# zhibaishouheilab/HealthiVert-GAN

Measured on NVIDIA B200. Metric: slices/sec two-stage gen fwd (256x256), higher is better.
Workload: dtype bf16

## Files before the change

### healthivert-gan_b200/build.py

```python
import os
import subprocess
import sys

HERE = os.path.dirname(os.path.abspath(__file__))
CSRC = os.path.join(HERE, "csrc")
LIB = os.path.join(HERE, "libhv_b200.so")
SOURCES = ["hv_api.cu", "sn_prepare.cu", "conv_fp32.cu", "ctx_attn.cu", "mask_ops.cu", "generator_plan.cu",
           "conv_tc.cu", "conv_tc_api.cu", "gemm_tc.cu", "ctx_attn_tc.cu", "train_ops.cu", "slice_prep.cu", "resample.cu", "pipeline.cu", "trunk_tc.cu", "dconv_tc.cu", "gconv_tc.cu"]
NVCC_FLAGS = ["-gencode", "arch=compute_100a,code=sm_100a", "-lineinfo", "-O3", "-std=c++17",
              "-Xcompiler", "-fPIC", "-shared"]


def _stale():
    if not os.path.exists(LIB):
        return True
    t = os.path.getmtime(LIB)
    deps = [os.path.join(CSRC, f) for f in os.listdir(CSRC)]
    deps.append(os.path.join(os.path.dirname(HERE), "include", "hv_b200.h"))
    return any(os.path.getmtime(d) > t for d in deps)


def build(force=False, verbose=False):
    if not force and not _stale():
        return LIB
    nvcc = os.environ.get("NVCC", "/usr/local/cuda/bin/nvcc")
    objs = []
    procs = []
    os.makedirs(os.path.join(HERE, "build"), exist_ok=True)
    for src in SOURCES:
        obj = os.path.join(HERE, "build", src.replace(".cu", ".o"))
        cmd = [nvcc] + NVCC_FLAGS[:-1] + ["-c", os.path.join(CSRC, src), "-o", obj]
        if verbose:
            cmd.insert(1, "-Xptxas=-v")
        procs.append((src, subprocess.Popen(cmd, stdout=subprocess.PIPE, stderr=subprocess.STDOUT, text=True)))
        objs.append(obj)
    for src, p in procs:
        out, _ = p.communicate()
        if verbose and out:
            print(out)
        if p.returncode != 0:
            raise RuntimeError(f"nvcc failed on {src}:\n{out}")
    cmd = [nvcc, "-gencode", "arch=compute_100a,code=sm_100a", "-shared", "-o", LIB] + objs
    r = subprocess.run(cmd, stdout=subprocess.PIPE, stderr=subprocess.STDOUT, text=True)
    if r.returncode != 0:
        raise RuntimeError(f"link failed:\n{r.stdout}")
    return LIB


if __name__ == "__main__":
    print(build(force="--force" in sys.argv, verbose="-v" in sys.argv))
```

### healthivert-gan_b200/csrc/conv_tc.cu

```cuda
#include <stdlib.h>
#include <string.h>
#include <vector>
#include "hv_common.cuh"
#include "conv_tc.cuh"
#include "tc_ptx.cuh"

namespace hv {

__device__ __forceinline__ float exp_neg_fast(float x) {
  float y;
  asm("ex2.approx.ftz.f32 %0, %1;" : "=f"(y) : "f"(x * 1.4426950408889634f));
  return y;
}

template <int ACT>
__device__ __forceinline__ float act_fast(float x, int act_rt) {
  if (ACT == HV_ACT_ELU) return x > 0.f ? x : exp_neg_fast(x) - 1.f;
  if (ACT == HV_ACT_RELU) return fmaxf(x, 0.f);
  switch (act_rt) {
    case HV_ACT_ELU: return x > 0.f ? x : __expf(x) - 1.f;
    case HV_ACT_RELU: return fmaxf(x, 0.f);
    case HV_ACT_SIGMOID: return 1.f / (1.f + __expf(-x));
    case HV_ACT_LRELU02: return x > 0.f ? x : 0.2f * x;
    case HV_ACT_CLAMP1: return fminf(fmaxf(x, -1.f), 1.f);
// ... 740 lines not shown
        const int ky = (ch >> 2) - py, kx = (ch & 3) - px;
        if (entry == 1 && ch < 16 && ky >= 0 && ky < 3 && kx >= 0 && kx < 3) v = wa[((size_t)co * cin_total + s.ch_off) * kk + ky * 3 + kx];
      } else if (ch < s.real) {
        const int dy = entry / 3 - 1, dx = entry % 3 - 1;
        for (int ky = 0; ky < 3; ++ky)
          for (int kx = 0; kx < 3; ++kx)
            if (((py + ky - 1) >> 1) == dy && ((px + kx - 1) >> 1) == dx) v += wa[((size_t)co * cin_total + s.ch_off + ch) * kk + ky * 3 + kx];
      }
    }
    dst[i] = __float2bfloat16(v);
    return;
  }
  if (real) {
    const int cin = s.ch_off + c;
    if (co < cout_a) v = wa[((size_t)co * cin_total + cin) * kk + tap];
    else if (co < cout_a + cout_b) v = wb[((size_t)(co - cout_a) * cin_total + cin) * kk + tap];
  }
  dst[i] = __float2bfloat16(v);
}

int tc_conv_pack_weights(TcConv& c, const float* wa, const float* ba, int cout_a, const float* wb, const float* bb,
                         int cout_b, cudaStream_t st) {
  HV_CHECK_ARG(cout_a + cout_b == c.cout_real, "tc_conv_pack_weights: filter count mismatch");
  PackSrc s0, s1;
  memset(&s0, 0, sizeof(s0)); memset(&s1, 0, sizeof(s1));
  s0.real = c.src[0].real_channels; s0.chunks = c.src[0].buf.chunks; s0.kxpack = c.src[0].kxpack ? 1 : 0; s0.xp = c.p.in_xp; s0.cp = c.p.cp;
  s1.chunks = 1; s1.xp = 1;
  s0.ups = c.p.ups;
  if (c.p.ups) HV_CHECK_ARG(cout_b == 0, "tc_conv_pack_weights: the sub-pixel upsample mode takes one filter bank");
  if (c.src[0].chan_map) {
    HV_CHECK_ARG(c.src[0].kxpack && c.src[0].buf.chunks * 8 <= 32, "tc_conv_pack_weights: a channel map needs a kx-packed source of <= 32 channels");
    s0.use_map = 1;
    for (int i = 0; i < 32; ++i) s0.map[i] = i < c.src[0].buf.chunks * 8 ? c.src[0].chan_map[i] : (short)-1;
  }
  int cin_total = c.src[0].real_channels;
  if (c.nsrc == 2) {
    s1.ch_off = c.src[0].real_channels; s1.real = c.src[1].real_channels; s1.chunks = c.src[1].buf.chunks; s1.kxpack = c.src[1].kxpack ? 1 : 0;
    s1.nbhd4 = c.src[1].nbhd4 ? 1 : 0;
    cin_total += c.src[1].real_channels;
  }
  const int total = (int)(c.p.w_bytes / 2);
  pack_weights_kernel<<<(max(total, c.n_pad) + 255) / 256, 256, 0, st>>>(wa, ba, cout_a, wb, bb, cout_b, cin_total, c.k, c.n_pad, s0,
                                                                          s1, c.nsrc, (__nv_bfloat16*)c.w_packed, c.bias_pad, total);
  HV_LAUNCH_CHECK();
  return HV_OK;
}

static long long* g_trace = nullptr;
static bool g_pdl = getenv("HV_NO_PDL") == nullptr;
void tc_set_trace(long long* dev_buf) { g_trace = dev_buf; }
static long long* g_timeline = nullptr;
static int g_timeline_count = 0;
void tc_set_timeline(long long* dev_buf) { g_timeline = dev_buf; g_timeline_count = 0; }

template <int N_PAD, int ACT, int FIXED = 0, bool DIAG = true>
static int tc_launch_na(const TcConv& c, cudaStream_t st) {
  static bool configured = false;
  if (!configured) {
    HV_CUDA(cudaFuncSetAttribute(conv_tc_kernel<N_PAD, ACT, FIXED, DIAG>, cudaFuncAttributeMaxDynamicSharedMemorySize, 227 * 1024));
    configured = true;
  }
  cudaLaunchConfig_t cfg = {};
  cfg.gridDim = dim3(c.grid);
  cfg.blockDim = dim3(tc_threads(N_PAD));
  cfg.dynamicSmemBytes = c.smem;
  cfg.stream = st;
  cudaLaunchAttribute attr[1];
  attr[0].id = cudaLaunchAttributeProgrammaticStreamSerialization;
  attr[0].val.programmaticStreamSerializationAllowed = 1;
  cfg.attrs = attr;
  cfg.numAttrs = g_pdl ? 1 : 0;
  TcParams q = c.p;
  q.trace = g_trace;
  q.timeline = g_timeline ? g_timeline + 4 * (g_timeline_count++) : nullptr;
  HV_CUDA(cudaLaunchKernelEx(&cfg, conv_tc_kernel<N_PAD, ACT, FIXED, DIAG>, q));
  HV_LAUNCH_CHECK();
  return HV_OK;
}

static int tc_issue_code(const TcConv& c);
static int tc_fixed_code(const TcConv& c) {
  if (c.force_generic) return 0;
  const int issue = tc_issue_code(c);
  if (!issue) return 0;
  const TcParams& p = c.p;
  int out = 0;
  if (p.out_mode == TC_OUT_HEADS) out = 3;
  else if (p.out_mode == TC_OUT_CHUNKED_S2D) out = 4;
  else if (p.out_mode == TC_OUT_CHUNKED) out = p.out_xp > 1 ? 5 : 1;
  else out = p.out_xp > 1 ? 6 : 2;
  return (p.pair ? 1 << 20 : 0) | out << 16 | issue;
}
static int tc_issue_code(const TcConv& c) {
  const TcParams& p = c.p;
  static const bool no_fixed = getenv("HV_TC_NO_FIXED") != nullptr;
  if (no_fixed) return 0;
  const TcSeg& s0 = p.segs[0];
  const int ks = s0.nchunks >> 1;
  if (p.s2d_in) return p.nseg == 1 ? tc_shape_code(2, 0, 0, ks) : 0;
  if (p.in_xp > 1) {
    for (int i = 1; i < p.nseg; ++i)
      if (p.segs[i].nrows != s0.nrows || p.segs[i].nchunks != s0.nchunks) return 0;
    return tc_shape_code(3, s0.nrows, 0, ks);
  }
  if (p.nseg == 2 && s0.nrows == 3 && s0.ntaps == 3 && p.segs[1].nrows == 3 && p.segs[1].ntaps == 1 && p.segs[1].nchunks == 2)
    return tc_shape_code(4, 0, 0, ks);
// ... 300 lines not shown
```

### healthivert-gan_b200/csrc/conv_tc.cuh

```cuda
#pragma once
#include <cuda.h>
#include <cuda_bf16.h>
#include <cuda_runtime.h>
#include <stdint.h>

namespace hv {

struct TcBuf {
  __nv_bfloat16* ptr = nullptr;
  int n = 0, chunks = 0, h = 0, w = 0, border = 0;
  bool s2d = false;
  int xp = 1;
  int img_chunks = 0;
  __host__ __device__ int image_chunks() const { return img_chunks ? img_chunks : chunks; }
  __host__ __device__ size_t chunk_base(int i, int c) const { return ((size_t)i * image_chunks() + c) * (size_t)plane() * 8; }
  TcBuf chunk_view(int c0, int count) const {
    TcBuf v = *this;
    v.img_chunks = image_chunks();
    v.ptr = ptr + (size_t)c0 * plane() * 8;
    v.chunks = count;
    return v;
  }
  __host__ __device__ int sub_h() const { return s2d ? h / 2 : h; }
  __host__ __device__ int sub_w() const { return s2d ? w / 2 : w / xp; }
// ... 60 lines not shown
  int out_mode;
  __nv_bfloat16* out;
  int out_pitch, out_border, out_plane, out_sub_plane, out_chunks_total, out_chunk_off, out_nchunks;
  float* head0;
  float* head1;
  TcAux aux0, aux1;
  uint32_t slot_bytes;
  int nslots;
  long long* trace;
  long long* timeline;
  int debug;
};

struct TcSource {
  TcBuf buf;
  int real_channels;
  bool kxpack = false;
  const short* chan_map = nullptr;
  bool nbhd4 = false;
};

struct TcConv {
  TcParams p;
  int n_pad = 0;
  int grid = 0;
  int ctas_per_sm = 1;
  size_t smem = 0;
  void* w_packed = nullptr;
  float* bias_pad = nullptr;
  int k = 0, stride = 1, dil = 1;
  int nsrc = 0;
  TcSource src[2];
  int cout_real = 0;
  bool force_generic = false;
  void* arena = nullptr;
  static constexpr size_t kArenaBytes = 4u << 20;
};

int tc_conv_setup(TcConv& c, const TcSource* srcs, int nsrc, int k, int stride, int dil, int cout_real,
                  int n_images, bool allow_pair = false, bool ups = false);
void tc_conv_set_batch(TcConv& c, int n_images);
int tc_conv_pack_weights(TcConv& c, const float* w_eff_a, const float* bias_a, int cout_a, const float* w_eff_b,
                         const float* bias_b, int cout_b, cudaStream_t st);
void tc_conv_set_output_chunked(TcConv& c, const TcBuf& out, int chunk_off, int nchunks, bool up2, int act);
void tc_conv_set_output_heads(TcConv& c, float* head0, float* head1, const TcAux* aux0, const TcAux* aux1);
int tc_conv_launch(const TcConv& c, cudaStream_t st);
void tc_set_trace(long long* dev_buf);
void tc_conv_free(TcConv& c);

bool tc_trunk_eligible(const TcConv& c);
size_t tc_trunk_counter_ints(int max_images);
int tc_trunk_launch(const TcConv* const* convs, int count, int n_images, int* counters, cudaStream_t st);

int tc_pack_nchw(const float* src, int src_channels, int mode , const TcBuf& dst, int dst_channel0,
                 cudaStream_t st);
struct TcPlaneSrc { const float* ptr; int mode; };
int tc_pack_kx(const TcPlaneSrc* srcs, int nsrc, int k, int dil, const TcBuf& dst, cudaStream_t st);
int tc_pack_nbhd4(const float* src, const TcBuf& dst, cudaStream_t st);
int tc_unpack_nchw(const TcBuf& src, int channel0, int channels, float* dst, cudaStream_t st, int sub = 1);
int tc_gap_fc_sigmoid(const TcBuf& x, const float* fc_w, const float* fc_b, float* out, float* partial ,
                      unsigned int* ticket , cudaStream_t st);

void tc_set_timeline(long long* dev_buf);
size_t ctx_attn_tc_workspace_bytes(int n);
int ctx_attn_fwd_tc(const TcBuf& f, const float* mask, const TcBuf& y, int32_t* offsets, float* flow, float scale, int fuse,
                    int per_sample_mask, void* workspace, cudaStream_t st, cudaStream_t st_aux = nullptr, cudaEvent_t* evs = nullptr);

}
```

### healthivert-gan_b200/csrc/generator_plan.cu

```cuda
#include <string.h>
#include <vector>
#include "hv_common.cuh"
#include "kernels.h"
#include "conv_tc.cuh"

namespace hv {

struct LayerSpec {
  const char* name;
  int cin, cout, k, stride, pad, dil, act, hout;
};

static const LayerSpec kLayers[] = {
    {"coarse_generator.conv1", 3, 16, 5, 1, 2, 1, HV_ACT_ELU, 256},
    {"coarse_generator.conv2_downsample", 16, 32, 3, 2, 1, 1, HV_ACT_ELU, 128},
    {"coarse_generator.conv3", 32, 32, 3, 1, 1, 1, HV_ACT_ELU, 128},
    {"coarse_generator.conv4_downsample", 32, 64, 3, 2, 1, 1, HV_ACT_ELU, 64},
    {"coarse_generator.conv5", 64, 64, 3, 1, 1, 1, HV_ACT_ELU, 64},
    {"coarse_generator.conv6", 64, 64, 3, 1, 1, 1, HV_ACT_ELU, 64},
    {"coarse_generator.conv7_atrous", 64, 64, 3, 1, 2, 2, HV_ACT_ELU, 64},
    {"coarse_generator.conv8_atrous", 64, 64, 3, 1, 4, 4, HV_ACT_ELU, 64},
    {"coarse_generator.conv9_atrous", 64, 64, 3, 1, 8, 8, HV_ACT_ELU, 64},
    {"coarse_generator.conv10_atrous", 64, 64, 3, 1, 16, 16, HV_ACT_ELU, 64},
    {"coarse_generator.conv11", 64, 64, 3, 1, 1, 1, HV_ACT_ELU, 64},
// ... 177 lines not shown
    {32, 128, 1}, {16, 128, 1}, {32, 256, 1}, {16, 256, 1}, {16, 256, 1},
    {32, 256, 2}, {32, 256, 1}, {16, 128, 1}, {32, 128, 1}, {32, 64, 1}, {64, 64, 1}, {64, 64, 2}, {64, 64, 4},
    {64, 64, 8}, {64, 64, 16}, {64, 64, 1},
    {0, 256, 1}, {16, 128, 1}, {32, 128, 1}, {64, 64, 1}, {64, 64, 1}, {64, 64, 1}, {64, 64, 1}, {64, 64, 1}, {64, 64, 1},
    {64, 64, 1}, {64, 64, 1}, {64, 64, 1}, {32, 128, 1}, {32, 128, 1}, {16, 256, 1}, {16, 256, 1},
};

struct TcLayerSpec { int layer; int src0, real0, src1, real1; int out; bool up2; int out_chunks; bool kx0, kx1; bool ups; };
static const TcLayerSpec kTcLayers[] = {
    {C1, B_IN_C, 3, -1, 0, B_C1, false, 2, true, false},  {C2, B_C1, 16, -1, 0, B_C2, false, 4},
    {C3, B_C2, 32, -1, 0, B_C3, false, 4},      {C4, B_C3, 32, -1, 0, B_C4, false, 8},
    {C5, B_C4, 64, -1, 0, B_C5, false, 8},      {C6, B_C5, 64, -1, 0, B_C6, false, 8},
    {C7, B_C6, 64, -1, 0, B_C7, false, 8},      {C8, B_C7, 64, -1, 0, B_C8, false, 8},
    {C9, B_C8, 64, -1, 0, B_C9, false, 8},      {C10, B_C9, 64, -1, 0, B_C10, false, 8},
    {C11, B_C10, 64, -1, 0, B_C11, false, 8},   {C12, B_C11, 64, -1, 0, B_C12U, true, 8},
    {C20, B_C12U, 64, B_CAM128, 1, B_C20, false, 8, false, true}, {C13, B_C20, 64, -1, 0, B_C13, false, 4},
    {C14, B_C13, 32, -1, 0, B_C14, false, 4},   {C19, B_C14, 32, B_CAM4, 1, B_C19, false, 4, false, true, true},
    {C15, B_C19, 32, -1, 0, B_C15, false, 2},   {C16, B_C15, 16, -1, 0, B_C16, false, 2},
    {C17, B_C16, 8, -1, 0, -1, false, 0},
    {F1, B_IN_F, 4, -1, 0, B_F1, false, 4, true, false},  {F2, B_F1, 16, -1, 0, B_F2, false, 2},
    {F3, B_F2, 16, -1, 0, B_F3, false, 4},      {F4, B_F3, 32, -1, 0, B_F4, false, 4},
    {F5, B_F4, 32, -1, 0, B_F5, false, 8},      {F6, B_F5, 64, -1, 0, B_F6, false, 8},
    {F7, B_F6, 64, -1, 0, B_F7, false, 8},      {F8, B_F7, 64, -1, 0, B_F8, false, 8},
    {F9, B_F8, 64, -1, 0, B_F9, false, 8},      {F10, B_F9, 64, -1, 0, B_F10, false, 8},
    {PM2, B_P1, 16, -1, 0, B_P2, false, 2},
    {PM3, B_P2, 16, -1, 0, B_P3, false, 4},     {PM4, B_P3, 32, -1, 0, B_P4, false, 8},
    {PM5, B_P4, 64, -1, 0, B_P5, false, 8},     {PM6, B_P5, 64, -1, 0, B_P6, false, 8},
    {PM9, B_CA, 64, -1, 0, B_P9, false, 8},     {PM10, B_P9, 64, -1, 0, B_P10, false, 8},
    {A11, B_F10, 64, B_P10, 64, B_A11, false, 8}, {A12, B_A11, 64, -1, 0, B_A12, false, 8},
    {A19, B_A12, 64, -1, 0, B_A19, false, 8},   {A13, B_A19, 64, -1, 0, B_A13, false, 4, false, false, true},
    {A14, B_A13, 32, -1, 0, B_A14, false, 4},   {A15, B_A14, 32, -1, 0, B_A15, false, 2, false, false, true},
    {A16, B_A15, 16, -1, 0, B_A16CAT, false, 1},
    {A17, B_A16CAT, 9, -1, 0, -1, false, 0},
};
constexpr int kNumTcLayers = sizeof(kTcLayers) / sizeof(kTcLayers[0]);

static const short kFineInputMap[32] = {
    0 * 64 + 0, 0 * 64 + 2, 0 * 64 + 3, 1 * 64 + 0, 1 * 64 + 2, 1 * 64 + 3, 2 * 64 + 0, 2 * 64 + 2, 2 * 64 + 3, 3 * 64 + 0, 3 * 64 + 2, 3 * 64 + 3,
    4 * 64 + 0, 4 * 64 + 2, 4 * 64 + 3, -1,
    0 * 64 + 1, 1 * 64 + 1, 2 * 64 + 1, 3 * 64 + 1, 4 * 64 + 1, -1, -1, -1, -1, -1, -1, -1, -1, -1, -1, -1};

struct TcPlan {
  TcBuf buf[B_COUNT];
  TcConv conv[kNumLayers];
  bool has[kNumLayers] = {};
  int out_buf[kNumLayers];
  bool out_up2[kNumLayers] = {};
  void* ca_ws = nullptr;
  float* gap_partial = nullptr;
  unsigned int* gap_ticket = nullptr;
  __nv_bfloat16* blob = nullptr;
  int* trunk_ctr = nullptr;
  size_t trunk_ctr_stride = 0;
};

static int run_layers(hv_generator* g, const int* layers, int count, int n, cudaStream_t st) {
  TcPlan* t = g->tc;
  static const int force = getenv("HV_TRUNK") ? atoi(getenv("HV_TRUNK")) : 0;
  static const int min_batch = getenv("HV_TRUNK_MIN_BATCH") ? atoi(getenv("HV_TRUNK_MIN_BATCH")) : (1 << 30);
  bool ok = (force == 1 || n >= min_batch) && count >= 2 && count <= 8;
  const TcConv* convs[8];
  for (int i = 0; i < count; ++i) {
    tc_conv_set_batch(t->conv[layers[i]], n);
    if (ok) { convs[i] = &t->conv[layers[i]]; ok = tc_trunk_eligible(*convs[i]) && (i == count - 1 || !t->out_up2[layers[i]]); }
  }
  if (ok) return tc_trunk_launch(convs, count, n, t->trunk_ctr + (size_t)layers[0] * t->trunk_ctr_stride, st);
  for (int i = 0; i < count; ++i) {
    int rc = tc_conv_launch(t->conv[layers[i]], st);
    if (rc) return rc;
  }
  return HV_OK;
}

static TcAux make_aux(const TcBuf& b, int channel) {
  TcAux a;
  a.ptr = b.ptr; a.chunks = b.chunks; a.chunk = channel >> 3; a.channel = channel & 7;
  a.pitch = b.pitch(); a.border = b.border; a.plane = b.plane(); a.sub_plane = b.sub_plane();
  return a;
}

static void tc_plan_destroy(hv_generator* g) {
  if (!g->tc) return;
  for (int i = 0; i < kNumLayers; ++i) if (g->tc->has[i]) tc_conv_free(g->tc->conv[i]);
  cudaFree(g->tc->blob); cudaFree(g->tc->ca_ws); cudaFree(g->tc->gap_partial); cudaFree(g->tc->gap_ticket); cudaFree(g->tc->trunk_ctr);
  delete g->tc;
  g->tc = nullptr;
}

static int tc_plan_create(hv_generator* g) {
  TcPlan* t = new TcPlan();
  g->tc = t;
  const int n = g->max_batch;
  size_t total = 0;
  const bool no_xp = getenv("HV_NO_XP") != nullptr;
  for (int i = 0; i < B_COUNT; ++i) {
    TcBuf& b = t->buf[i];
    b.n = n; b.chunks = kBufs[i].channels / 8; b.h = b.w = kBufs[i].extent; b.border = kBufs[i].border;
    b.s2d = (i == B_C1 || i == B_C3 || i == B_F1 || i == B_F3 || i == B_P1 || i == B_P3);
    b.xp = (!no_xp && (i == B_C19 || i == B_C15 || i == B_C16 || i == B_A15 || i == B_A16CAT)) ? 4 : 1;
    total += (b.bytes() + 255) & ~(size_t)255;
  }
  total += TcBuf::kSlackBytes;
  HV_CUDA(cudaMalloc((void**)&t->blob, total));
  HV_CUDA(cudaMemset(t->blob, 0, total));
  size_t off = 0;
  for (int i = 0; i < B_COUNT; ++i) {
    t->buf[i].ptr = reinterpret_cast<__nv_bfloat16*>(reinterpret_cast<char*>(t->blob) + off);
    off += (t->buf[i].bytes() + 255) & ~(size_t)255;
  }
  t->buf[B_P1] = t->buf[B_F1].chunk_view(2, 2);
  HV_CUDA(cudaMalloc(&t->ca_ws, ctx_attn_tc_workspace_bytes(n)));
  HV_CUDA(cudaMalloc((void**)&t->gap_partial, sizeof(float) * 2 * n * 8));
  HV_CUDA(cudaMalloc((void**)&t->gap_ticket, sizeof(unsigned int) * 2 * n));
  HV_CUDA(cudaMemset(t->gap_ticket, 0, sizeof(unsigned int) * 2 * n));
  t->trunk_ctr_stride = tc_trunk_counter_ints(n);
  HV_CUDA(cudaMalloc((void**)&t->trunk_ctr, sizeof(int) * t->trunk_ctr_stride * kNumLayers));
  HV_CUDA(cudaMemset(t->trunk_ctr, 0, sizeof(int) * t->trunk_ctr_stride * kNumLayers));
  for (int i = 0; i < kNumLayers; ++i) t->out_buf[i] = -1;
  t->out_buf[PM1] = B_P1;
  for (int i = 0; i < kNumTcLayers; ++i) {
    const TcLayerSpec& s = kTcLayers[i];
    const LayerSpec& L = kLayers[s.layer];
    TcSource srcs[2];
    srcs[0].buf = s.layer == F2 ? t->buf[B_F1].chunk_view(0, 2) : t->buf[s.src0];
    srcs[0].real_channels = s.real0; srcs[0].kxpack = s.kx0;
    if (s.layer == F1) srcs[0].chan_map = kFineInputMap;
    int nsrc = 1;
    if (s.src1 >= 0) { srcs[1].buf = t->buf[s.src1]; srcs[1].real_channels = s.real1; srcs[1].kxpack = s.kx1; srcs[1].nbhd4 = s.ups; nsrc = 2; }
    const bool heads = s.out < 0;
    TcConv& c = t->conv[s.layer];
    const int cout = heads ? 2 : (s.layer == F1 ? kLayers[F1].cout + kLayers[PM1].cout : L.cout);
    int rc = tc_conv_setup(c, srcs, nsrc, L.k, L.stride, L.dil, cout, n, true, s.ups);
    if (rc) return rc;
    t->has[s.layer] = true;
    if (heads) {
      TcAux a0 = make_aux(t->buf[B_A16CAT], 8);
      tc_conv_set_output_heads(c, nullptr, nullptr, s.layer == C17 ? &a0 : nullptr, nullptr);
    } else {
      tc_conv_set_output_chunked(c, t->buf[s.out], 0, s.out_chunks, s.up2, L.act);
      t->out_buf[s.layer] = s.out; t->out_up2[s.layer] = s.up2;
    }
  }
  return HV_OK;
}

static void tc_set_batch(TcConv& c, int n) { tc_conv_set_batch(c, n); }

static int tc_plan_pack_weights(hv_generator* g, cudaStream_t st) {
  TcPlan* t = g->tc;
  for (int i = 0; i < kNumTcLayers; ++i) {
    const int l = kTcLayers[i].layer;
    int rc;
    if (kTcLayers[i].out < 0)
      rc = tc_conv_pack_weights(t->conv[l], g->w_eff[l], g->bias[l], 1, g->w_eff[l + 1], g->bias[l + 1], 1, st);
    else if (l == F1)
      rc = tc_conv_pack_weights(t->conv[l], g->w_eff[F1], g->bias[F1], kLayers[F1].cout, g->w_eff[PM1], g->bias[PM1], kLayers[PM1].cout, st);
    else
      rc = tc_conv_pack_weights(t->conv[l], g->w_eff[l], g->bias[l], kLayers[l].cout, nullptr, nullptr, 0, st);
    if (rc) return rc;
  }
  return HV_OK;
}

static int forward_bf16(hv_generator* g, const float* x, const float* mask, const float* cam, const float* ratio, int n,
                        float* coarse_seg, float* fine_seg, float* x_stage1, float* x_stage2, float* flow, float* pred1_h,
                        float* pred2_h, int32_t* offsets, int per_sample_mask, cudaStream_t st) {
  TcPlan* t = g->tc;
  auto view = [&](int id) { TcBuf b = t->buf[id]; b.n = n; return b; };
  auto run = [&](int layer, cudaStream_t s) -> int {
    TcConv& c = t->conv[layer];
    tc_set_batch(c, n);
    return tc_conv_launch(c, s);
  };
  static const bool use_aux = getenv("HV_NO_AUX_STREAM") == nullptr;
  cudaStream_t ax = use_aux ? g->aux : st;
  auto fork_aux = [&](int ev) -> int {
    if (!use_aux) return HV_OK;
    HV_CUDA(cudaEventRecord(g->ev_aux[ev], st));
    HV_CUDA(cudaStreamWaitEvent(ax, g->ev_aux[ev], 0));
    return HV_OK;
  };
  auto join_aux = [&](int ev) -> int {
    if (!use_aux) return HV_OK;
    HV_CUDA(cudaEventRecord(g->ev_aux[ev], ax));
    HV_CUDA(cudaStreamWaitEvent(st, g->ev_aux[ev], 0));
    return HV_OK;
  };
  {
    RC(fork_aux(0));
    const TcPlaneSrc in_c[3] = {{x, HV_SRC_DIRECT}, {ratio, HV_SRC_SCALAR}, {mask, HV_SRC_DIRECT}};
    RC(tc_pack_kx(in_c, 3, 5, 1, view(B_IN_C), st));
    const TcPlaneSrc cam128[1] = {{cam, HV_SRC_SUB2}};
    RC(tc_pack_kx(cam128, 1, 3, 1, view(B_CAM128), ax));
    RC(tc_pack_nbhd4(cam, view(B_CAM4), ax));
    const TcPlaneSrc in_f0[3] = {{x, HV_SRC_DIRECT}, {mask, HV_SRC_DIRECT}, {ratio, HV_SRC_SCALAR}};
    RC(tc_pack_kx(in_f0, 3, 5, 1, view(B_IN_F).chunk_view(0, 2), ax));
    if (use_aux) HV_CUDA(cudaEventRecord(g->ev_aux[1], ax));
  }
  auto chain = [&](std::initializer_list<int> ls, cudaStream_t s) -> int { return run_layers(g, ls.begin(), (int)ls.size(), n, s); };
  for (int l : {C1, C2, C3, C4}) RC(run(l, st));
  RC(chain({C5, C6, C7, C8, C9, C10, C11, C12}, st));
  RC(fork_aux(2));
  RC(tc_gap_fc_sigmoid(view(B_C10), g->fc_w[0], g->fc_b[0], pred1_h, t->gap_partial, t->gap_ticket, ax));
  if (use_aux) HV_CUDA(cudaStreamWaitEvent(st, g->ev_aux[1], 0));
  for (int l : {C20, C13, C14, C19, C15, C16}) RC(run(l, st));
  t->conv[C17].p.head0 = x_stage1; t->conv[C17].p.head1 = coarse_seg;
  RC(run(C17, st));
  {
    const TcPlaneSrc in_f1[1] = {{coarse_seg, HV_SRC_DIRECT}};
    RC(tc_pack_kx(in_f1, 1, 5, 1, view(B_IN_F).chunk_view(2, 2), st));
  }
  RC(run(F1, st));
  HV_CUDA(cudaEventRecord(g->ev_fork, st));
  HV_CUDA(cudaStreamWaitEvent(g->side, g->ev_fork, 0));
  cudaStream_t sa = g->side;
  for (int l : {PM2, PM3, PM4}) RC(run(l, sa));
  RC(chain({PM5, PM6}, sa));
  RC(ctx_attn_fwd_tc(view(B_P6), mask, view(B_CA), offsets, flow, 10.f, 1, per_sample_mask, t->ca_ws, sa, use_aux ? ax : nullptr,
                     use_aux ? &g->ev_aux[6] : nullptr));
  RC(chain({PM9, PM10}, sa));
  HV_CUDA(cudaEventRecord(g->ev_join, sa));
  for (int l : {F2, F3, F4, F5}) RC(run(l, st));
  RC(chain({F6, F7, F8, F9, F10}, st));
  HV_CUDA(cudaStreamWaitEvent(st, g->ev_join, 0));
  RC(run(A11, st));
  RC(fork_aux(4));
  RC(tc_gap_fc_sigmoid(view(B_A11), g->fc_w[1], g->fc_b[1], pred2_h, t->gap_partial + g->max_batch * 8, t->gap_ticket + g->max_batch, ax));
  RC(chain({A12, A19}, st));
  for (int l : {A13, A14, A15, A16}) RC(run(l, st));
  t->conv[A17].p.head0 = x_stage2; t->conv[A17].p.head1 = fine_seg;
  RC(run(A17, st));
  RC(join_aux(5));
  g->last_heads[0] = x_stage1; g->last_heads[1] = coarse_seg; g->last_heads[2] = x_stage2; g->last_heads[3] = fine_seg;
  g->last_n = n;
  return HV_OK;
}

}

extern "C" {

int hv_generator_num_layers(void) { return kNumLayers; }

int hv_generator_layer_info(int idx, char* name_out, int* cin, int* cout, int* k, int* stride, int* pad, int* dil,
                            int* act) {
  HV_CHECK_ARG(idx >= 0 && idx < kNumLayers, "layer_info: index %d out of range", idx);
  const LayerSpec& L = kLayers[idx];
  if (name_out) { strncpy(name_out, L.name, 63); name_out[63] = 0; }
  if (cin) *cin = L.cin;
  if (cout) *cout = L.cout;
  if (k) *k = L.k;
  if (stride) *stride = L.stride;
  if (pad) *pad = L.pad;
  if (dil) *dil = L.dil;
  if (act) *act = L.act;
  return HV_OK;
}

int hv_generator_destroy(hv_generator* g) {
  if (!g) return HV_OK;
  tc_plan_destroy(g);
  for (int i = 0; i < kNumLayers; ++i) cudaFree(g->act[i]);
  cudaFree(g->ca_out); cudaFree(g->ca_ws); cudaFree(g->sigma); cudaFree(g->d_jobs);
  cudaFree(g->blob_w); cudaFree(g->blob_b);
  if (g->side) cudaStreamDestroy(g->side);
  if (g->ev_fork) cudaEventDestroy(g->ev_fork);
  if (g->ev_join) cudaEventDestroy(g->ev_join);
  if (g->aux) cudaStreamDestroy(g->aux);
  for (cudaEvent_t e : g->ev_aux) if (e) cudaEventDestroy(e);
  delete g;
  return HV_OK;
}

int hv_generator_create(hv_generator** out, int max_batch, int precision) {
  HV_CHECK_ARG(out, "generator_create: null out pointer");
  HV_CHECK_ARG(max_batch >= 1 && max_batch <= 4096, "generator_create: max_batch %d out of range", max_batch);
  HV_CHECK_ARG(precision == HV_PREC_FP32 || precision == HV_PREC_BF16, "generator_create: bad precision %d", precision);
  int ndev = 0;
  HV_CUDA(cudaGetDeviceCount(&ndev));
  hv_generator* g = new hv_generator();
  g->max_batch = max_batch; g->precision = precision;
  size_t wtot = 0, btot = 0;
  for (int i = 0; i < kNumLayers; ++i) { wtot += (size_t)kLayers[i].cout * kLayers[i].cin * kLayers[i].k * kLayers[i].k; btot += kLayers[i].cout; }
#define GEN_TRY(expr) do { cudaError_t _e = (expr); if (_e != cudaSuccess) { hv::set_error("%s failed: %s", #expr, cudaGetErrorString(_e)); hv_generator_destroy(g); return HV_ERR_CUDA; } } while (0)
// ... 76 lines not shown
    return forward_bf16(g, x, mask, cam, ratio, n, coarse_seg, fine_seg, x_stage1, x_stage2, flow, pred1_h, pred2_h,
                        offsets, per_sample_mask, as_stream(stream));
  return forward_fp32(g, x, mask, cam, ratio, n, coarse_seg, fine_seg, x_stage1, x_stage2, flow, pred1_h, pred2_h,
                      offsets, per_sample_mask, as_stream(stream));
}

int hv_generator_run_layer(hv_generator* g, int idx, int n, hv_stream_t stream) {
  HV_CHECK_ARG(g && g->tc, "generator_run_layer: needs a bf16 plan");
  if (!g->prepared) { set_error("generator_run_layer: call hv_generator_prepare first"); return HV_ERR_STATE; }
  HV_CHECK_ARG(idx >= 0 && idx < kNumLayers && g->tc->has[idx] && g->tc->out_buf[idx] >= 0,
               "generator_run_layer: layer %d is not a stand-alone tensor-core conv", idx);
  HV_CHECK_ARG(n >= 1 && n <= g->max_batch, "generator_run_layer: batch %d outside 1..%d", n, g->max_batch);
  tc_set_batch(g->tc->conv[idx], n);
  return tc_conv_launch(g->tc->conv[idx], as_stream(stream));
}

int hv_generator_run_chain(hv_generator* g, int first, int count, int n, hv_stream_t stream) {
  HV_CHECK_ARG(g && g->tc, "generator_run_chain: needs a bf16 plan");
  if (!g->prepared) { set_error("generator_run_chain: call hv_generator_prepare first"); return HV_ERR_STATE; }
  HV_CHECK_ARG(n >= 1 && n <= g->max_batch && count >= 1 && first >= 0 && first + count <= kNumLayers, "generator_run_chain: bad range");
  int layers[kNumLayers];
  for (int idx = first; idx < first + count; ++idx) {
    HV_CHECK_ARG(g->tc->has[idx] && g->tc->out_buf[idx] >= 0, "generator_run_chain: layer %d is not a stand-alone tensor-core conv", idx);
    layers[idx - first] = idx;
  }
  return run_layers(g, layers, count, n, as_stream(stream));
}

long long hv_generator_read_tap(hv_generator* g, int idx, float* out, hv_stream_t stream) {
  HV_CHECK_ARG(g && out, "generator_read_tap: null argument");
  HV_CHECK_ARG(g->last_n > 0, "generator_read_tap: no forward has run");
  const float* src = nullptr;
  size_t count = 0;
  if (idx == kTapAttention && g->tc) {
    TcBuf v = g->tc->buf[B_CA];
    v.n = g->last_n;
    int rc = tc_unpack_nchw(v, 0, 64, out, as_stream(stream));
    if (rc) return rc;
    return (long long)g->last_n * 64 * 64 * 64;
  }
  if (idx == kTapAttention) { src = g->ca_out; count = (size_t)g->last_n * 64 * 64 * 64; }
  else {
    HV_CHECK_ARG(idx >= 0 && idx < kNumLayers, "generator_read_tap: index %d out of range", idx);
    count = act_elems(idx, g->last_n);
    if (idx == C17) src = g->last_heads[0];
    else if (idx == C18) src = g->last_heads[1];
    else if (idx == A17) src = g->last_heads[2];
    else if (idx == A18) src = g->last_heads[3];
    else if (g->tc) {
      const int b = g->tc->out_buf[idx];
      HV_CHECK_ARG(b >= 0, "generator_read_tap: layer %d has no tap in bf16 mode", idx);
      TcBuf v = g->tc->buf[b];
      v.n = g->last_n;
      const int ch = idx == A16 ? 8 : kLayers[idx].cout;
      int rc = tc_unpack_nchw(v, 0, ch, out, as_stream(stream), g->tc->out_up2[idx] ? 2 : 1);
      if (rc) return rc;
      return (long long)count;
    }
    else src = g->act[idx];
  }
  HV_CUDA(cudaMemcpyAsync(out, src, count * sizeof(float), cudaMemcpyDeviceToDevice, as_stream(stream)));
  return (long long)count;
}

}
```

Baseline: 20520.

## Fuse final 3x3 conv and dual heads into one warp-specialized tcgen05 tail kernel

Adds a persistent tail kernel that computes the last mid 3x3 ELU conv and the dual-head 3x3 conv (tanh-clamp and sigmoid) back to back. The intermediate activation stays in shared memory ring slots instead of going through global memory. The kernel also writes the kx-packed coarse segmentation for the refinement stage, which removes the separate pack_kx launch. Both stages of the generator use it by default. Tap reads of the fused mid layers now recompute them on demand, and the tight pipeline adds synchronization complexity and correctness risk.

```diff
diff --git a/healthivert-gan_b200/build.py b/healthivert-gan_b200/build.py
--- a/healthivert-gan_b200/build.py
+++ b/healthivert-gan_b200/build.py
@@ -6,7 +6,7 @@
 CSRC = os.path.join(HERE, "csrc")
 LIB = os.path.join(HERE, "libhv_b200.so")
 SOURCES = ["hv_api.cu", "sn_prepare.cu", "conv_fp32.cu", "ctx_attn.cu", "mask_ops.cu", "generator_plan.cu",
-           "conv_tc.cu", "conv_tc_api.cu", "gemm_tc.cu", "ctx_attn_tc.cu", "train_ops.cu", "slice_prep.cu", "resample.cu", "pipeline.cu", "trunk_tc.cu", "dconv_tc.cu", "gconv_tc.cu"]
+           "conv_tc.cu", "conv_tc_api.cu", "gemm_tc.cu", "ctx_attn_tc.cu", "train_ops.cu", "slice_prep.cu", "resample.cu", "pipeline.cu", "trunk_tc.cu", "tail_tc.cu", "dconv_tc.cu", "gconv_tc.cu"]
 NVCC_FLAGS = ["-gencode", "arch=compute_100a,code=sm_100a", "-lineinfo", "-O3", "-std=c++17",
               "-Xcompiler", "-fPIC", "-shared"]
 
diff --git a/healthivert-gan_b200/csrc/conv_tc.cu b/healthivert-gan_b200/csrc/conv_tc.cu
--- a/healthivert-gan_b200/csrc/conv_tc.cu
+++ b/healthivert-gan_b200/csrc/conv_tc.cu
@@ -816,6 +816,8 @@
 static long long* g_timeline = nullptr;
 static int g_timeline_count = 0;
 void tc_set_timeline(long long* dev_buf) { g_timeline = dev_buf; g_timeline_count = 0; }
+bool tc_pdl_enabled() { return g_pdl; }
+long long* tc_timeline_next() { return g_timeline ? g_timeline + 4 * (g_timeline_count++) : nullptr; }
 
 template <int N_PAD, int ACT, int FIXED = 0, bool DIAG = true>
 static int tc_launch_na(const TcConv& c, cudaStream_t st) {
diff --git a/healthivert-gan_b200/csrc/conv_tc.cuh b/healthivert-gan_b200/csrc/conv_tc.cuh
--- a/healthivert-gan_b200/csrc/conv_tc.cuh
+++ b/healthivert-gan_b200/csrc/conv_tc.cuh
@@ -136,6 +136,33 @@
 size_t tc_trunk_counter_ints(int max_images);
 int tc_trunk_launch(const TcConv* const* convs, int count, int n_images, int* counters, cudaStream_t st);
 
+struct TcTailParams {
+  CUtensorMap maps[4];
+  const void* w_mid;
+  const void* w_head;
+  const float* bias_mid;
+  const float* bias_head;
+  int n, h, w_img;
+  int rows_per_unit, strips, units;
+  float* head0;
+  float* head1;
+  TcAux aux0;
+  TcBuf kx;
+  int kx_chunk;
+  long long* timeline;
+};
+struct TcTail {
+  TcTailParams p;
+  int grid = 0;
+};
+int tc_tail_setup(TcTail& t, const TcConv& mid, const TcConv& heads, int n_images);
+void tc_tail_set_batch(TcTail& t, int n_images);
+void tc_tail_set_outputs(TcTail& t, float* head0, float* head1);
+int tc_tail_set_kxpack(TcTail& t, const TcBuf* dst, int chunk);
+int tc_tail_launch(const TcTail& t, cudaStream_t st);
+bool tc_pdl_enabled();
+long long* tc_timeline_next();
+
 int tc_pack_nchw(const float* src, int src_channels, int mode , const TcBuf& dst, int dst_channel0,
                  cudaStream_t st);
 struct TcPlaneSrc { const float* ptr; int mode; };
diff --git a/healthivert-gan_b200/csrc/generator_plan.cu b/healthivert-gan_b200/csrc/generator_plan.cu
--- a/healthivert-gan_b200/csrc/generator_plan.cu
+++ b/healthivert-gan_b200/csrc/generator_plan.cu
@@ -253,7 +253,14 @@
   __nv_bfloat16* blob = nullptr;
   int* trunk_ctr = nullptr;
   size_t trunk_ctr_stride = 0;
-};
+  TcTail tail[2];
+  bool tail_fused_last = false;
+};
+
+static bool tail_fuse_enabled() {
+  static const bool on = !(getenv("HV_NO_TAIL_FUSE") && atoi(getenv("HV_NO_TAIL_FUSE")) != 0) && !getenv("HV_NO_XP");
+  return on;
+}
 
 static int run_layers(hv_generator* g, const int* layers, int count, int n, cudaStream_t st) {
   TcPlan* t = g->tc;
@@ -341,6 +348,12 @@
       tc_conv_set_output_chunked(c, t->buf[s.out], 0, s.out_chunks, s.up2, L.act);
       t->out_buf[s.layer] = s.out; t->out_up2[s.layer] = s.up2;
     }
+  }
+  if (tail_fuse_enabled()) {
+    int rc = tc_tail_setup(t->tail[0], t->conv[C16], t->conv[C17], n);
+    if (!rc) rc = tc_tail_setup(t->tail[1], t->conv[A16], t->conv[A17], n);
+    if (!rc) rc = tc_tail_set_kxpack(t->tail[0], &t->buf[B_IN_F], 2);
+    if (rc) return rc;
   }
   return HV_OK;
 }
@@ -404,10 +417,20 @@
   RC(fork_aux(2));
   RC(tc_gap_fc_sigmoid(view(B_C10), g->fc_w[0], g->fc_b[0], pred1_h, t->gap_partial, t->gap_ticket, ax));
   if (use_aux) HV_CUDA(cudaStreamWaitEvent(st, g->ev_aux[1], 0));
-  for (int l : {C20, C13, C14, C19, C15, C16}) RC(run(l, st));
-  t->conv[C17].p.head0 = x_stage1; t->conv[C17].p.head1 = coarse_seg;
-  RC(run(C17, st));
-  {
+  const bool fuse_tail = tail_fuse_enabled();
+  auto tail = [&](int which, int conv, int heads, float* head0, float* head1) -> int {
+    if (fuse_tail) {
+      tc_tail_set_batch(t->tail[which], n);
+      tc_tail_set_outputs(t->tail[which], head0, head1);
+      return tc_tail_launch(t->tail[which], st);
+    }
+    RC(run(conv, st));
+    t->conv[heads].p.head0 = head0; t->conv[heads].p.head1 = head1;
+    return run(heads, st);
+  };
+  for (int l : {C20, C13, C14, C19, C15}) RC(run(l, st));
+  RC(tail(0, C16, C17, x_stage1, coarse_seg));
+  if (!fuse_tail) {
     const TcPlaneSrc in_f1[1] = {{coarse_seg, HV_SRC_DIRECT}};
     RC(tc_pack_kx(in_f1, 1, 5, 1, view(B_IN_F).chunk_view(2, 2), st));
   }
@@ -428,9 +451,9 @@
   RC(fork_aux(4));
   RC(tc_gap_fc_sigmoid(view(B_A11), g->fc_w[1], g->fc_b[1], pred2_h, t->gap_partial + g->max_batch * 8, t->gap_ticket + g->max_batch, ax));
   RC(chain({A12, A19}, st));
-  for (int l : {A13, A14, A15, A16}) RC(run(l, st));
-  t->conv[A17].p.head0 = x_stage2; t->conv[A17].p.head1 = fine_seg;
-  RC(run(A17, st));
+  for (int l : {A13, A14, A15}) RC(run(l, st));
+  RC(tail(1, A16, A17, x_stage2, fine_seg));
+  t->tail_fused_last = fuse_tail;
   RC(join_aux(5));
   g->last_heads[0] = x_stage1; g->last_heads[1] = coarse_seg; g->last_heads[2] = x_stage2; g->last_heads[3] = fine_seg;
   g->last_n = n;
@@ -613,6 +636,11 @@
       HV_CHECK_ARG(b >= 0, "generator_read_tap: layer %d has no tap in bf16 mode", idx);
       TcBuf v = g->tc->buf[b];
       v.n = g->last_n;
+      if (g->tc->tail_fused_last && (idx == C16 || idx == A16)) {
+        tc_set_batch(g->tc->conv[idx], g->last_n);
+        int rc = tc_conv_launch(g->tc->conv[idx], as_stream(stream));
+        if (rc) return rc;
+      }
       const int ch = idx == A16 ? 8 : kLayers[idx].cout;
       int rc = tc_unpack_nchw(v, 0, ch, out, as_stream(stream), g->tc->out_up2[idx] ? 2 : 1);
       if (rc) return rc;
diff --git a/healthivert-gan_b200/csrc/tail_tc.cu b/healthivert-gan_b200/csrc/tail_tc.cu
--- /dev/null
+++ b/healthivert-gan_b200/csrc/tail_tc.cu
@@ -0,0 +1,418 @@
+#include <string.h>
+#include "hv_common.cuh"
+#include "conv_tc.cuh"
+#include "tc_ptx.cuh"
+
+namespace hv {
+
+namespace {
+
+constexpr int kMidN = 32, kHeadN = 16;
+constexpr uint32_t kWMid = 3u * 6u * 2u * kMidN * 16u;
+constexpr uint32_t kWHead = 3u * 6u * 2u * kHeadN * 16u;
+constexpr uint32_t kSlot = 6u * 2u * 2u * 64u * 16u;
+constexpr int kSlots = 4;
+constexpr uint32_t kOffIn = kWMid + kWHead;
+constexpr uint32_t kOffMid = kOffIn + kSlots * kSlot;
+constexpr uint32_t kOffBar = kOffMid + kSlots * kSlot;
+constexpr uint32_t kOffKx = kOffBar + 1024;
+constexpr int kKxRow = 264;
+constexpr uint32_t kSmem = kOffKx + 2u * 2u * kKxRow * 4u;
+static_assert(kSmem <= 227u * 1024u, "tail kernel shared memory");
+constexpr uint32_t kInTx = kSlot;
+constexpr uint32_t kAuxTx = kSlot / 2;
+constexpr int kThreads = 20 * 32;
+constexpr int kTmemCols = 128;
+
+__device__ __forceinline__ float elu_fast(float x) {
+  if (x > 0.f) return x;
+  float y;
+  asm("ex2.approx.ftz.f32 %0, %1;" : "=f"(y) : "f"(x * 1.4426950408889634f));
+  return y - 1.f;
+}
+
+template <int N>
+__device__ __forceinline__ void issue_rows(bool leader, uint32_t d_tmem, const uint32_t (&a_lo)[3], uint32_t a_view, uint32_t b_lo) {
+  constexpr uint32_t desc_hi = (128u >> 4) | (1u << 14);
+  constexpr uint32_t idesc = (1u << 4) | (1u << 7) | (1u << 10) | ((uint32_t)(N >> 3) << 17) | ((128u >> 4) << 24);
+  constexpr uint32_t slab = 2u * N;
+  if (leader) {
+#pragma unroll
+    for (int ky = 0; ky < 3; ++ky)
+#pragma unroll
+      for (int v = 0; v < 6; ++v)
+        umma_bf16(d_tmem, ((uint64_t)desc_hi << 32) | (a_lo[ky] + (uint32_t)v * a_view),
+                  ((uint64_t)desc_hi << 32) | (b_lo + (uint32_t)(ky * 6 + v) * slab), idesc, (ky | v) == 0 ? 0u : 1u);
+  }
+}
+
+}
+
+__global__ void __launch_bounds__(kThreads, 1) tail_tc_kernel(const __grid_constant__ TcTailParams p) {
+  extern __shared__ __align__(1024) uint8_t smem[];
+  const int warp = threadIdx.x >> 5, lane = threadIdx.x & 31;
+  constexpr int W_PRODUCER = 16, W_MMA = 17, W_HEADS = 18, W_AUX = 19;
+  const uint32_t s_base = smem_u32(smem);
+  const uint32_t bars = s_base + kOffBar;
+  const uint32_t bar_in_full = bars, bar_in_empty = bars + 8 * kSlots;
+  const uint32_t bar_mid_ready = bars + 16 * kSlots, bar_mid_free = bars + 24 * kSlots;
+  const uint32_t bar_mfull = bars + 32 * kSlots, bar_mempty = bar_mfull + 16, bar_hfull = bar_mfull + 32, bar_hempty = bar_mfull + 48;
+  const uint32_t bar_w = bar_mfull + 64;
+  uint32_t* tmem_slot = reinterpret_cast<uint32_t*>(smem + kOffBar + 256);
+  float* s_bias = reinterpret_cast<float*>(smem + kOffBar + 512);
+
+  if (p.timeline && threadIdx.x == 0) {
+    unsigned long long gt;
+    asm volatile("mov.u64 %0, %%globaltimer;" : "=l"(gt));
+    atomicMin(reinterpret_cast<unsigned long long*>(p.timeline), gt);
+  }
+  if ((warp == W_PRODUCER || warp == W_AUX) && lane == 0) {
+    for (int i = 0; i < 4; ++i) asm volatile("prefetch.tensormap [%0];" ::"l"(&p.maps[i]) : "memory");
+  }
+  if (warp == W_MMA) {
+    if (lane == 0) {
+      for (int i = 0; i < kSlots; ++i) {
+        mbar_init(bar_in_full + 8u * i, 1);
+        mbar_init(bar_in_empty + 8u * i, 1);
+        mbar_init(bar_mid_ready + 8u * i, 128 + 1);
+        mbar_init(bar_mid_free + 8u * i, 1);
+      }
+      for (int i = 0; i < 2; ++i) {
+        mbar_init(bar_mfull + 8u * i, 1); mbar_init(bar_mempty + 8u * i, 128);
+        mbar_init(bar_hfull + 8u * i, 1); mbar_init(bar_hempty + 8u * i, 128);
+      }
+      mbar_init(bar_w, 1);
+      fence_barrier_init();
+    }
+    __syncwarp();
+    asm volatile("tcgen05.alloc.cta_group::1.sync.aligned.shared::cta.b32 [%0], %1;" ::"r"(smem_u32(tmem_slot)), "r"(kTmemCols) : "memory");
+    asm volatile("tcgen05.relinquish_alloc_permit.cta_group::1.sync.aligned;" ::: "memory");
+  }
+  if (threadIdx.x < kMidN) s_bias[threadIdx.x] = __ldg(p.bias_mid + threadIdx.x);
+  else if (threadIdx.x < kMidN + kHeadN) s_bias[threadIdx.x] = __ldg(p.bias_head + threadIdx.x - kMidN);
+  if (threadIdx.x < kSlots * 2 * 2) {
+    const int slot = threadIdx.x >> 2, s = (threadIdx.x >> 1) & 1, e = threadIdx.x & 1;
+    *reinterpret_cast<uint4*>(smem + kOffMid + slot * kSlot + (e ? 5 * 2048 + s * 1024 + 63 * 16 : s * 1024)) = make_uint4(0, 0, 0, 0);
+    fence_proxy_async();
+  }
+  if (threadIdx.x >= 64 && threadIdx.x < 64 + 2 * 2 * 8) {
+    const int r = (threadIdx.x - 64) >> 3, e = (threadIdx.x - 64) & 7;
+    reinterpret_cast<float*>(smem + kOffKx)[r * kKxRow + (e < 4 ? e : kKxRow - 8 + e)] = 0.f;
+  }
+  tc_fence_before();
+  __syncthreads();
+  tc_fence_after();
+  const uint32_t tmem_base = *tmem_slot;
+  asm volatile("griddepcontrol.launch_dependents;" ::: "memory");
+
+  const int R = p.rows_per_unit, strips = p.strips, units = p.units, h = p.h;
+
+  if (warp == W_PRODUCER || warp == W_AUX) {
+    const bool leader = elect_one();
+    const bool in_role = warp == W_PRODUCER;
+    if (leader && in_role) {
+      mbar_expect_tx(bar_w, kWMid + kWHead);
+      bulk_load(s_base, p.w_mid, kWMid, bar_w);
+      bulk_load(s_base + kWMid, p.w_head, kWHead, bar_w);
+    }
+    asm volatile("griddepcontrol.wait;" ::: "memory");
+    uint32_t in_seq = 0, mid_seq = 0;
+    for (int u = blockIdx.x; u < units; u += gridDim.x) {
+      const int pair = u / strips, y0 = (u - pair * strips) * R, ru = min(R, h - y0), img = 2 * pair;
+      for (int i = -2; i <= ru + 1; ++i) {
+        if (in_role) {
+          const uint32_t slot = in_seq % kSlots, par = (in_seq / kSlots) & 1u;
+          mbar_wait(bar_in_empty + 8u * slot, par ^ 1u);
+          if (leader) {
+            const uint32_t fb = bar_in_full + 8u * slot, dst = s_base + kOffIn + slot * kSlot;
+            const int row = y0 + i + 1;
+            mbar_expect_tx(fb, kInTx);
+            tma_load_5d(dst + 4096u, &p.maps[0], fb, 2, img, row, 0, 0);
+            tma_load_5d(dst, &p.maps[1], fb, 0, img, row, 0, 3);
+            tma_load_5d(dst + 5u * 4096u, &p.maps[1], fb, 4, img, row, 0, 0);
+          }
+          ++in_seq;
+        }
+        const int j = i - 1;
+        if (!in_role && j >= -1) {
+          const uint32_t slot = mid_seq % kSlots, par = (mid_seq / kSlots) & 1u;
+          mbar_wait(bar_mid_free + 8u * slot, par ^ 1u);
+          if (leader) {
+            const uint32_t fb = bar_mid_ready + 8u * slot, dst = s_base + kOffMid + slot * kSlot + 12288u;
+            const int row = y0 + j + 1;
+            mbar_expect_tx(fb, kAuxTx);
+            tma_load_5d(dst + 2048u, &p.maps[2], fb, 2, img, row, 1, 0);
+            tma_load_5d(dst, &p.maps[3], fb, 0, img, row, 1, 3);
+            tma_load_5d(dst + 5u * 2048u, &p.maps[3], fb, 4, img, row, 1, 0);
+          }
+          ++mid_seq;
+        }
+      }
+    }
+  } else if (warp == W_MMA || warp == W_HEADS) {
+    const bool leader = elect_one();
+    const bool conv_role = warp == W_MMA;
+    mbar_wait(bar_w, 0);
+    tc_fence_after();
+    const uint32_t b_mid = ((uint32_t)kMidN << 16) + (s_base >> 4);
+    const uint32_t b_head = ((uint32_t)kHeadN << 16) + ((s_base + kWMid) >> 4);
+    const uint32_t a_in = ((2048u >> 4) << 16) + ((s_base + kOffIn) >> 4);
+    const uint32_t a_mid = ((12288u >> 4) << 16) + ((s_base + kOffMid) >> 4);
+    uint32_t in_base = 0, mid_base = 0, waited = 0, cnt = 0;
+    for (int u = blockIdx.x; u < units; u += gridDim.x) {
+      const int pair = u / strips, y0 = (u - pair * strips) * R, ru = min(R, h - y0);
+      if (conv_role) {
+        for (int j = -1; j <= ru; ++j, ++cnt) {
+          while (waited < in_base + (uint32_t)(j + 4)) {
+            mbar_wait(bar_in_full + 8u * (waited % kSlots), (waited / kSlots) & 1u);
+            ++waited;
+          }
+          const uint32_t acc = cnt & 1u;
+          mbar_wait(bar_mempty + 8u * acc, ((cnt >> 1) & 1u) ^ 1u);
+          tc_fence_after();
+          uint32_t a_lo[3];
+#pragma unroll
+          for (int ky = 0; ky < 3; ++ky) a_lo[ky] = a_in + ((in_base + (uint32_t)(j + 1 + ky)) % kSlots) * (kSlot >> 4);
+          issue_rows<kMidN>(leader, tmem_base + acc * kMidN, a_lo, 4096u >> 4, b_mid);
+          if (leader) {
+            umma_commit(bar_mfull + 8u * acc);
+            umma_commit(bar_in_empty + 8u * ((in_base + (uint32_t)(j + 1)) % kSlots));
+            if (j == ru) {
+              umma_commit(bar_in_empty + 8u * ((in_base + (uint32_t)(j + 2)) % kSlots));
+              umma_commit(bar_in_empty + 8u * ((in_base + (uint32_t)(j + 3)) % kSlots));
+            }
+          }
+          __syncwarp();
+        }
+      } else {
+        for (int k = 0; k < ru; ++k, ++cnt) {
+          while (waited < mid_base + (uint32_t)(k + 3)) {
+            mbar_wait(bar_mid_ready + 8u * (waited % kSlots), (waited / kSlots) & 1u);
+            ++waited;
+          }
+          const uint32_t acc = cnt & 1u;
+          mbar_wait(bar_hempty + 8u * acc, ((cnt >> 1) & 1u) ^ 1u);
+          tc_fence_after();
+          uint32_t a_lo[3];
+#pragma unroll
+          for (int ky = 0; ky < 3; ++ky) a_lo[ky] = a_mid + ((mid_base + (uint32_t)(k + ky)) % kSlots) * (kSlot >> 4);
+          issue_rows<kHeadN>(leader, tmem_base + 2 * kMidN + acc * kHeadN, a_lo, 2048u >> 4, b_head);
+          if (leader) {
+            umma_commit(bar_hfull + 8u * acc);
+            umma_commit(bar_mid_free + 8u * ((mid_base + (uint32_t)k) % kSlots));
+            if (k == ru - 1) {
+              umma_commit(bar_mid_free + 8u * ((mid_base + (uint32_t)(k + 1)) % kSlots));
+              umma_commit(bar_mid_free + 8u * ((mid_base + (uint32_t)(k + 2)) % kSlots));
+            }
+          }
+          __syncwarp();
+        }
+      }
+      in_base += (uint32_t)(ru + 4);
+      mid_base += (uint32_t)(ru + 2);
+    }
+  } else {
+    const int quad = warp & 3, m = quad * 32 + lane, s = m >> 6, q = m & 63;
+    const uint32_t lane_off = (uint32_t)(quad * 32) << 16;
+    const bool mid_role = warp < 8;
+    const uint32_t group = (uint32_t)((warp >> 2) & 1);
+    uint32_t cnt = 0;
+    for (int u = blockIdx.x; u < units; u += gridDim.x) {
+      const int pair = u / strips, y0 = (u - pair * strips) * R, ru = min(R, h - y0);
+      const int img = 2 * pair + s;
+      if (mid_role) {
+        for (int j = -1; j <= ru; ++j, ++cnt) {
+          if ((cnt & 1u) != group) continue;
+          mbar_wait(bar_mfull + 8u * group, (cnt >> 1) & 1u);
+          tc_fence_after();
+          float v[kMidN];
+          tmem_ld<32>(tmem_base + lane_off + group * kMidN, v);
+          tmem_ld_wait();
+          tc_fence_before();
+          mbar_arrive(bar_mempty + 8u * group);
+          const int y = y0 + j;
+          const bool inside = y >= 0 && y < h;
+          uint4 val[4];
+#pragma unroll
+          for (int ph = 0; ph < 4; ++ph) {
+            uint32_t pk[4];
+#pragma unroll
+            for (int e = 0; e < 4; ++e) {
+              const int col = ph * 8 + 2 * e;
+              __nv_bfloat162 hv2 = __floats2bfloat162_rn(elu_fast(v[col] + s_bias[col]), elu_fast(v[col + 1] + s_bias[col + 1]));
+              pk[e] = inside ? *reinterpret_cast<uint32_t*>(&hv2) : 0u;
+            }
+            val[ph] = make_uint4(pk[0], pk[1], pk[2], pk[3]);
+          }
+          const uint32_t slot = cnt % kSlots;
+          mbar_wait(bar_mid_free + 8u * slot, ((cnt / kSlots) & 1u) ^ 1u);
+          uint8_t* base = smem + kOffMid + slot * kSlot + s * 1024 + q * 16;
+#pragma unroll
+          for (int ph = 0; ph < 4; ++ph) *reinterpret_cast<uint4*>(base + (ph + 1) * 2048) = val[ph];
+          if (q < 63) *reinterpret_cast<uint4*>(base + 16) = val[3];
+          if (q > 0) *reinterpret_cast<uint4*>(base + 5 * 2048 - 16) = val[0];
+          fence_proxy_async();
+          mbar_arrive(bar_mid_ready + 8u * slot);
+        }
+      } else {
+        for (int k = 0; k < ru; ++k, ++cnt) {
+          if ((cnt & 1u) != group) continue;
+          mbar_wait(bar_hfull + 8u * group, (cnt >> 1) & 1u);
+          tc_fence_after();
+          float v[kHeadN];
+          tmem_ld<16>(tmem_base + lane_off + 2 * kMidN + group * kHeadN, v);
+          tmem_ld_wait();
+          tc_fence_before();
+          mbar_arrive(bar_hempty + 8u * group);
+          const bool live = img < p.n;
+          const int y = y0 + k;
+          float seg[4];
+#pragma unroll
+          for (int jx = 0; jx < 4; ++jx) {
+            const int x = 4 * q + jx;
+            const float a0 = fminf(fmaxf(v[jx * 4] + s_bias[kMidN + jx * 4], -1.f), 1.f);
+            const float a1 = 1.f / (1.f + __expf(-(v[jx * 4 + 1] + s_bias[kMidN + jx * 4 + 1])));
+            seg[jx] = a1;
+            if (!live) continue;
+            const size_t pix = ((size_t)img * h + y) * p.w_img + x;
+            p.head0[pix] = a0;
+            p.head1[pix] = a1;
+            if (p.aux0.ptr) {
+              const TcAux& a = p.aux0;
+              const size_t pos = (size_t)jx * a.sub_plane + (size_t)(y + a.border) * a.pitch + q + a.border;
+              a.ptr[(((size_t)img * a.chunks + a.chunk) * a.plane + pos) * 8 + a.channel] = __float2bfloat16(a0);
+            }
+          }
+          if (p.kx.ptr) {
+            float* row = reinterpret_cast<float*>(smem + kOffKx) + (group * 2 + s) * kKxRow;
+            *reinterpret_cast<float4*>(row + 4 + 4 * q) = make_float4(seg[0], seg[1], seg[2], seg[3]);
+            asm volatile("bar.sync %0, 128;" ::"r"(1 + (int)group) : "memory");
+            if (live) {
+              __nv_bfloat16* dst = p.kx.ptr + p.kx.chunk_base(img, p.kx_chunk) + p.kx.pos(y, 4 * q) * 8;
+#pragma unroll
+              for (int jx = 0; jx < 4; ++jx) {
+                const float* r = row + 2 + 4 * q + jx;
+                __nv_bfloat162 c01 = __floats2bfloat162_rn(r[0], r[1]), c23 = __floats2bfloat162_rn(r[2], r[3]);
+                __nv_bfloat162 c4 = __floats2bfloat162_rn(r[4], 0.f);
+                *reinterpret_cast<uint4*>(dst + jx * 8) = make_uint4(*reinterpret_cast<uint32_t*>(&c01), *reinterpret_cast<uint32_t*>(&c23),
+                                                                     *reinterpret_cast<uint32_t*>(&c4), 0u);
+              }
+            }
+            asm volatile("bar.sync %0, 128;" ::"r"(1 + (int)group) : "memory");
+          }
+        }
+      }
+    }
+  }
+  tc_fence_before();
+  __syncthreads();
+  if (p.timeline && threadIdx.x == 0) {
+    unsigned long long gt;
+    asm volatile("mov.u64 %0, %%globaltimer;" : "=l"(gt));
+    atomicMax(reinterpret_cast<unsigned long long*>(p.timeline) + 1, gt);
+  }
+  if (warp == W_MMA) {
+    tc_fence_after();
+    asm volatile("tcgen05.dealloc.cta_group::1.sync.aligned.b32 %0, %1;" ::"r"(tmem_base), "r"(kTmemCols) : "memory");
+  }
+}
+
+typedef CUresult (*PFN_encodeTiledTail)(CUtensorMap*, CUtensorMapDataType, cuuint32_t, void*, const cuuint64_t*, const cuuint64_t*,
+                                        const cuuint32_t*, const cuuint32_t*, CUtensorMapInterleave, CUtensorMapSwizzle,
+                                        CUtensorMapL2promotion, CUtensorMapFloatOOBfill);
+
+static int make_tail_map(CUtensorMap* map, const TcBuf& b, int box_chunks, int box_phases) {
+  void* ptr = nullptr;
+  cudaDriverEntryPointQueryResult qres;
+  if (cudaGetDriverEntryPoint("cuTensorMapEncodeTiled", &ptr, cudaEnableDefault, &qres) != cudaSuccess || qres != cudaDriverEntryPointSuccess) {
+    set_error("cuTensorMapEncodeTiled is unavailable (driver entry point lookup failed)");
+    return HV_ERR_CUDA;
+  }
+  PFN_encodeTiledTail enc = reinterpret_cast<PFN_encodeTiledTail>(ptr);
+  const cuuint64_t sub_b = (cuuint64_t)b.sub_plane() * 16, plane_b = (cuuint64_t)b.plane() * 16;
+  cuuint64_t dims[5] = {(cuuint64_t)b.pitch() * 2, (cuuint64_t)b.n, (cuuint64_t)b.rows(), (cuuint64_t)b.image_chunks(), 4};
+  cuuint64_t strides[4] = {plane_b * b.image_chunks(), (cuuint64_t)b.pitch() * 16, plane_b, sub_b};
+  cuuint32_t box[5] = {128, 2, 1, (cuuint32_t)box_chunks, (cuuint32_t)box_phases};
+  cuuint32_t es[5] = {1, 1, 1, 1, 1};
+  CUresult r = enc(map, CU_TENSOR_MAP_DATA_TYPE_UINT64, 5, b.ptr, dims, strides, box, es, CU_TENSOR_MAP_INTERLEAVE_NONE,
+                   CU_TENSOR_MAP_SWIZZLE_NONE, CU_TENSOR_MAP_L2_PROMOTION_L2_256B, CU_TENSOR_MAP_FLOAT_OOB_FILL_NONE);
+  if (r != CUDA_SUCCESS) { set_error("tail: cuTensorMapEncodeTiled failed with CUresult %d", (int)r); return HV_ERR_CUDA; }
+  return HV_OK;
+}
+
+int tc_tail_setup(TcTail& t, const TcConv& mid, const TcConv& heads, int n_images) {
+  const TcBuf& in = mid.src[0].buf;
+  const TcBuf& hb = heads.src[0].buf;
+  HV_CHECK_ARG(mid.nsrc == 1 && mid.k == 3 && mid.dil == 1 && mid.p.in_xp == 4 && mid.n_pad == kMidN && in.chunks == 2 && in.sub_w() == 64,
+               "tc_tail: the first layer must be a 16 -> 8 x-phase 3x3 conv over 256-pixel rows");
+  HV_CHECK_ARG(mid.p.out_mode == TC_OUT_CHUNKED && mid.p.act == HV_ACT_ELU, "tc_tail: the first layer must be a chunked ELU conv");
+  HV_CHECK_ARG(heads.nsrc == 1 && heads.k == 3 && heads.p.in_xp == 4 && heads.n_pad == kHeadN && heads.p.out_mode == TC_OUT_HEADS &&
+                   hb.chunks == 2 && hb.h == in.h && hb.w == in.w && hb.border == 1 && in.border == 1,
+               "tc_tail: the second layer must be the dual heads over a 2-chunk x-phase buffer of the same geometry");
+  HV_CHECK_ARG(mid.p.w_bytes == kWMid && heads.p.w_bytes == kWHead, "tc_tail: unexpected packed weight sizes");
+  t.p = TcTailParams();
+  int rc = make_tail_map(&t.p.maps[0], in, 2, 4);
+  if (!rc) rc = make_tail_map(&t.p.maps[1], in, 2, 1);
+  if (!rc) rc = make_tail_map(&t.p.maps[2], hb, 1, 4);
+  if (!rc) rc = make_tail_map(&t.p.maps[3], hb, 1, 1);
+  if (rc) return rc;
+  t.p.w_mid = mid.w_packed; t.p.w_head = heads.w_packed;
+  t.p.bias_mid = mid.bias_pad; t.p.bias_head = heads.bias_pad;
+  t.p.h = in.h; t.p.w_img = in.w;
+  t.p.aux0 = heads.p.aux0;
+  tc_tail_set_batch(t, n_images);
+  return HV_OK;
+}
+
+void tc_tail_set_batch(TcTail& t, int n_images) {
+  static int sms = 0;
+  if (!sms) {
+    int dev = 0;
+    cudaGetDevice(&dev);
+    if (cudaDeviceGetAttribute(&sms, cudaDevAttrMultiProcessorCount, dev) != cudaSuccess || sms <= 0) sms = 148;
+  }
+  const int pairs = (n_images + 1) / 2, h = t.p.h;
+  const int want_strips = max(1, min(h, sms / pairs));
+  const int rows = (h + want_strips - 1) / want_strips;
+  t.p.n = n_images;
+  t.p.rows_per_unit = rows;
+  t.p.strips = (h + rows - 1) / rows;
+  t.p.units = pairs * t.p.strips;
+  t.grid = min(t.p.units, sms);
+}
+
+void tc_tail_set_outputs(TcTail& t, float* head0, float* head1) { t.p.head0 = head0; t.p.head1 = head1; }
+
+int tc_tail_set_kxpack(TcTail& t, const TcBuf* dst, int chunk) {
+  if (!dst) { t.p.kx = TcBuf(); return HV_OK; }
+  HV_CHECK_ARG(dst->ptr && dst->xp == 1 && !dst->s2d && dst->h == t.p.h && dst->w == t.p.w_img && chunk >= 0 && chunk < dst->image_chunks(),
+               "tc_tail_set_kxpack: destination must be a plain chunked buffer of the heads' extent");
+  t.p.kx = *dst;
+  t.p.kx_chunk = chunk;
+  return HV_OK;
+}
+
+int tc_tail_launch(const TcTail& t, cudaStream_t st) {
+  static bool configured = false;
+  if (!configured) {
+    HV_CUDA(cudaFuncSetAttribute(tail_tc_kernel, cudaFuncAttributeMaxDynamicSharedMemorySize, (int)kSmem));
+    configured = true;
+  }
+  cudaLaunchConfig_t cfg = {};
+  cfg.gridDim = dim3(t.grid);
+  cfg.blockDim = dim3(kThreads);
+  cfg.dynamicSmemBytes = kSmem;
+  cfg.stream = st;
+  cudaLaunchAttribute attr[1];
+  attr[0].id = cudaLaunchAttributeProgrammaticStreamSerialization;
+  attr[0].val.programmaticStreamSerializationAllowed = 1;
+  cfg.attrs = attr;
+  cfg.numAttrs = tc_pdl_enabled() ? 1 : 0;
+  TcTailParams q = t.p;
+  q.timeline = tc_timeline_next();
+  HV_CUDA(cudaLaunchKernelEx(&cfg, tail_tc_kernel, q));
+  HV_LAUNCH_CHECK();
+  return HV_OK;
+}
+
+}
```

Measured after the change: 21150 (median of 6 runs). 3.1% higher.
